# quantummind/mpi_opt

Measured on AMD Instinct MI355X. Metric: EI candidates/sec (GP/EI ask step, N=200 obs, D=10, fp64), higher is better.
Workload: dtype f64; 1 GPU; BASELINE configs[1]: GP/EI ask step, 200 observations, 10-dim, 1000000 candidates per GPU, top-5 (skopt argsort[:n_restarts]); n_obs=200, dims=10, candidates_per_gpu=1000000, parallelism=candidates sharded, 1 GPU(s), all-gather of (value,index)

## Files before the change

mpi_opt_amd/csrc/gp.hip:

```cpp

#include "mpo_internal.h"

#include <algorithm>
#include <cmath>
#include <cstdlib>
#include <string>

namespace {

typedef double f64x4 __attribute__((ext_vector_type(4)));

constexpr double kSqrt5 = 2.236067977499789696409173668731276235;
constexpr double kSqrt1_2 = 0.707106781186547524400844362104849039;
constexpr double kSqrt2Pi = 2.506628274631000502415765284811045253;
constexpr double kJitter = 1e-10;

__device__ __forceinline__ double matern52(double r, double amp) {
    const double k = r * kSqrt5;
    return amp * ((1.0 + k + k * k * (1.0 / 3.0)) * exp(-k));
}

__device__ __forceinline__ double fma_sc(double a, double b, double c) {
    double r;
    asm("v_fma_f64 %0, %1, %2, %3" : "=v"(r) : "v"(a), "v"(b), "s"(c));
// ... 146 lines not shown
        double xx = 0.0;
        for (int c = 0; c < d; ++c) xx = fma(xs[(size_t)i * dp + c], xs[(size_t)i * dp + c], xx);
        for (int c = 0; c < dp; ++c)
            xb[(size_t)i * dp + c] = c < d ? -2.0 * xs[(size_t)i * dp + c] : c == d ? 1.0 : c == d + 1 ? xx : 0.0;
        if (!(xx <= kDistNorm)) atomicOr(&bad, 1);
    }
    __syncthreads();
    if (threadIdx.x == 0) xb[(size_t)rows * dp] = bad ? 0.0 : 1.0;
}

__global__ __launch_bounds__(256) void xb_check_kernel(const double* __restrict__ mqd, const double* __restrict__ mqm,
                                                       const double* __restrict__ alpha, int n, double amp,
                                                       double* __restrict__ flag) {
    __shared__ int bad;
    __shared__ double red[4];
    if (threadIdx.x == 0) bad = 0;
    double sa = 0.0;
    for (int i = threadIdx.x; i < n; i += 256) sa += fabs(alpha[i]);
    for (int o = 32; o > 0; o >>= 1) sa += __shfl_down(sa, o, 64);
    if ((threadIdx.x & 63) == 0) red[threadIdx.x >> 6] = sa;
    __syncthreads();
    const double mu_scale = amp * (red[0] + red[1] + red[2] + red[3]);
    for (int i = threadIdx.x; i < n; i += 256) {
        const double mud = mqd[2 * i], qd = mqd[2 * i + 1], mum = mqm[2 * i], qm = mqm[2 * i + 1];
        const bool ok = fabs(qm - qd) <= 1e-10 * fmax(amp - qd, 1e-300) && fabs(mum - mud) <= 1e-10 * mu_scale;
        if (!ok) atomicOr(&bad, 1);
    }
    __syncthreads();
    if (threadIdx.x == 0 && bad) flag[0] = 0.0;
}

__global__ void kernel_matrix_unscaled_kernel(const double* __restrict__ X, int n, int d,
                                              const double* __restrict__ ls, double amp,
                                              double diag_add, double* __restrict__ K, int ldk) {
    const int j = blockIdx.x * blockDim.x + threadIdx.x;
    const int i = blockIdx.y;
    if (j >= n) return;
    double r2 = 0.0;
    for (int c = 0; c < d; ++c) {
        const double t = X[(size_t)i * d + c] / ls[c] - X[(size_t)j * d + c] / ls[c];
        r2 += t * t;
    }
    double v = matern52(sqrt(r2), amp);
    if (i == j) v += diag_add;
    K[(size_t)i * ldk + j] = v;
}

__global__ __launch_bounds__(1024) void chol_kernel(double* __restrict__ A, int n, int lda,
                                                    int32_t* __restrict__ info) {
    __shared__ int fail;
    const int tid = threadIdx.x, nt = blockDim.x;
    const int lane = tid & 63, wave = tid >> 6, nwave = nt >> 6;
    if (tid == 0) fail = 0;
    __syncthreads();
    for (int j = 0; j < n; ++j) {
        if (tid == 0) {
            const double djj = A[(size_t)j * lda + j];
            if (!(djj > 0.0) || !isfinite(djj)) fail = j + 1;
            else A[(size_t)j * lda + j] = sqrt(djj);
        }
        __syncthreads();
        if (fail) break;
        const double ljj = A[(size_t)j * lda + j];
        for (int i = j + 1 + tid; i < n; i += nt) A[(size_t)i * lda + j] /= ljj;
        __syncthreads();
        for (int i = j + 1 + wave; i < n; i += nwave) {
            const double lij = A[(size_t)i * lda + j];
            for (int k = j + 1 + lane; k <= i; k += 64)
                A[(size_t)i * lda + k] -= lij * A[(size_t)k * lda + j];
        }
        __syncthreads();
    }
    if (tid == 0) *info = fail;
}

__global__ __launch_bounds__(64) void trsm_kernel(const double* __restrict__ L, int n, int lda,
                                                  double* __restrict__ B, int nrhs, int ldb,
                                                  int trans, int cb) {
    extern __shared__ __attribute__((aligned(16))) double xsol[];
    const int lc = threadIdx.x;
    const int col = blockIdx.x * cb + lc;
    const bool active = lc < cb && col < nrhs;
    if (!active) return;
    if (!trans) {
        for (int i = 0; i < n; ++i) {
            double s = B[(size_t)i * ldb + col];
            const double* Li = L + (size_t)i * lda;
            for (int k = 0; k < i; ++k) s -= Li[k] * xsol[k * cb + lc];
            const double x = s / Li[i];
            xsol[i * cb + lc] = x;
            B[(size_t)i * ldb + col] = x;
        }
    } else {
        for (int i = n - 1; i >= 0; --i) {
            double s = B[(size_t)i * ldb + col];
            for (int k = i + 1; k < n; ++k) s -= L[(size_t)k * lda + i] * xsol[k * cb + lc];
            const double x = s / L[(size_t)i * lda + i];
            xsol[i * cb + lc] = x;
            B[(size_t)i * ldb + col] = x;
        }
    }
}

constexpr int kStreamSlack = 2;
inline size_t wfrag_elems(int np16) {
    const size_t T = np16 / 16;
    return (T * (T + 1) / 2 + 4 * kStreamSlack) * 256;
}
inline size_t wmeta_elems(int np16) {
    const int T = np16 / 16;
    return (size_t)4 * (T + 4) + T + 4;
}

__global__ void wave_plan_kernel(int T, int32_t* __restrict__ meta) {
    if (threadIdx.x != 0 || blockIdx.x != 0) return;
    int load[4] = {0, 0, 0, 0}, cnt[4] = {0, 0, 0, 0};
    for (int jt = T - 1; jt >= 0; --jt) {
        int w = 0;
        for (int v = 1; v < 4; ++v)
            if (load[v] < load[w]) w = v;
        meta[w * (T + 4) + 3 + cnt[w]++] = jt;
        load[w] += jt + 1;
    }
    int off = 0;
    for (int w = 0; w < 4; ++w) {
        int32_t* r = meta + w * (T + 4);
        r[0] = off;
        r[1] = load[w];
        r[2] = cnt[w];
        for (int t = cnt[w]; t <= T; ++t) r[3 + t] = 0;
        int g = off;
        for (int t = 0; t < cnt[w]; ++t) {
            meta[4 * (T + 4) + r[3 + t]] = g;
            g += r[3 + t] + 1;
        }
        off += load[w] + kStreamSlack;
    }
}

__global__ void pack_wfrag_kernel(const double* __restrict__ W, int n, int ldw, int T,
                                  const int32_t* __restrict__ meta, double* __restrict__ wfrag) {
    const int jt = blockIdx.y;
    if (jt >= T) return;
    const int nks = 4 * (jt + 1);
    const int e = blockIdx.x * blockDim.x + threadIdx.x;
    if (e >= nks * 64) return;
    const int ks = e >> 6, l = e & 63;
    const int i = 4 * ks + (l >> 4), j = 16 * jt + (l & 15);
    const double v = (i < n && j < n && i <= j) ? W[(size_t)j * ldw + i] : 0.0;
    wfrag[(size_t)meta[4 * (T + 4) + jt] * 256 + e] = v;
}

constexpr int kBM = 16;

struct ScoreArgs {
    int n, np16, T, d;
    double amp, y_mean, y_std;
    const double* xs;
    const double* xb;
    const double* xb_ok;
    const double* ls;
    const double* alpha;
    const double* wfrag;
    const int32_t* wmeta;
    const double* cand;
    long long m;
    double y_opt, xi, kappa;
    unsigned flags;
    int ei_positive;
    int dbg;
    double* mu;
    double* sd;
    double* vals;
    int k;
    long long* part_idx;
    double* part_val;
    double* mq;
    int panel;
    double* part;
};

__device__ __attribute__((noinline)) void score_finish_group(const ScoreArgs& a, bool valid, long long gm, double mu_n,
                                                   double q, int lane, double* tk_val, long long* tk_idx) {
    double mu = 0.0, sd = 0.0, vei = 0.0, vpi = 0.0, vlcb = 0.0;
    if (valid && (a.dbg & 8)) {
        mu = mu_n;
        sd = q;
    } else if (valid) {
        double var = a.amp - q;
        if (var < 0.0) var = 0.0;
        sd = sqrt(var) * a.y_std;
        mu = a.y_std * mu_n + a.y_mean;
        if (sd > 0.0) {
            const double improve = a.y_opt - a.xi - mu;
            const double scaled = improve / sd;
            const double cdf = ndtr(scaled);
            vei = -(improve * cdf + sd * norm_pdf(scaled));
            vpi = -cdf;
        } else {
            vei = -0.0;
            vpi = -0.0;
        }
        vlcb = mu - a.kappa * sd;
        if (a.mu) a.mu[gm] = mu;
        if (a.sd) a.sd[gm] = sd;
        if (a.vals) {
            if (a.flags & MPO_ACQ_EI) a.vals[gm] = a.ei_positive ? -vei : vei;
            if (a.flags & MPO_ACQ_PI) a.vals[a.m + gm] = vpi;
            if (a.flags & MPO_ACQ_LCB) a.vals[2 * a.m + gm] = vlcb;
        }
    }
    if (a.k <= 0 || (a.dbg & 4)) return;
    const double inf = __builtin_huge_val();
    const long long big = 0x7fffffffffffffffLL;
    const int k = a.k;
#pragma unroll
    for (int acq = 0; acq < 3; ++acq) {
        if (!(a.flags & (1u << acq))) continue;
        const double v = valid ? (acq == 0 ? vei : (acq == 1 ? vpi : vlcb)) : inf;
        const long long idx = valid ? gm : big;
        double* lv = tk_val + acq * MPO_TOPK_MAX;
        long long* li = tk_idx + acq * MPO_TOPK_MAX;
        bool cand = valid && lex_less(v, idx, lv[k - 1], li[k - 1]);
        while (__any(cand)) {
            double bv = cand ? v : inf;
            long long bi = cand ? idx : big;
            wave_lex_min(bv, bi);
            if (lane == 0) {
                int pos = k - 1;
                while (pos > 0 && lex_less(bv, bi, lv[pos - 1], li[pos - 1])) {
                    lv[pos] = lv[pos - 1];
                    li[pos] = li[pos - 1];
                    --pos;
                }
                lv[pos] = bv;
                li[pos] = bi;
            }
            asm volatile("s_waitcnt lgkmcnt(0)" ::: "memory");
            cand = cand && idx != bi && lex_less(v, idx, lv[k - 1], li[k - 1]);
        }
    }
}

__device__ __forceinline__ void score_finish_own_rows(double* kc, int wave, int lane) {
    constexpr int BM = kBM;
    __syncthreads();
    const ScoreArgs* ap = (const ScoreArgs*)__builtin_amdgcn_kernarg_segment_ptr();
    asm volatile("" : "+s"(ap));
    const ScoreArgs& f = *ap;
    double* tk_val = kc + wave * 3 * MPO_TOPK_MAX;
    long long* tk_idx = reinterpret_cast<long long*>(kc + 4 * 3 * MPO_TOPK_MAX) + wave * 3 * MPO_TOPK_MAX;
    if (lane < 3 * MPO_TOPK_MAX) {
        tk_val[lane] = __builtin_huge_val();
        tk_idx[lane] = 0x7fffffffffffffffLL;
    }
    asm volatile("s_waitcnt lgkmcnt(0)" ::: "memory");
    const long long ntl = ((f.m + BM - 1) / BM - blockIdx.x + gridDim.x - 1) / gridDim.x;
    for (long long c0 = (long long)wave * 64; c0 < ntl * BM; c0 += 256) {
        const long long cl = c0 + lane;
        const long long gm = (blockIdx.x + (cl >> 4) * (long long)gridDim.x) * BM + (cl & 15);
        const bool valid = cl < ntl * BM && gm < f.m;
        double2 v = {0.0, 0.0};
        if (valid) v = *reinterpret_cast<const double2*>(f.mq + 2 * gm);
        score_finish_group(f, valid, gm, v.x, v.y, lane, tk_val, tk_idx);
    }
    if (f.k > 0 && lane < 3 * f.k) {
        const int acq = lane / f.k, r = lane - acq * f.k;
        const size_t part = (size_t)blockIdx.x * 4 + wave;
        f.part_val[(part * 3 + acq) * f.k + r] = tk_val[acq * MPO_TOPK_MAX + r];
        f.part_idx[(part * 3 + acq) * f.k + r] = tk_idx[acq * MPO_TOPK_MAX + r];
    }
}

#define MPO_LD(D, P, OFF) asm volatile("global_load_dwordx2 %0, %1, off offset:" #OFF : "=v"(D) : "v"(P) : "memory")
#define MPO_LD4(B, P) { MPO_LD(B[0], P, 0); MPO_LD(B[1], P, 512); MPO_LD(B[2], P, 1024); MPO_LD(B[3], P, 1536); }
#define MPO_MFMA4(AP, B0, B1, B2, B3)                                                              \
    acc0 = __builtin_amdgcn_mfma_f64_16x16x4f64((AP)[0], B0, acc0, 0, 0, 0);                       \
    acc1 = __builtin_amdgcn_mfma_f64_16x16x4f64((AP)[64], B1, acc1, 0, 0, 0);                      \
    acc0 = __builtin_amdgcn_mfma_f64_16x16x4f64((AP)[128], B2, acc0, 0, 0, 0);                     \
    acc1 = __builtin_amdgcn_mfma_f64_16x16x4f64((AP)[192], B3, acc1, 0, 0, 0);
#define MPO_EI_PAIR(XC, AC, LI)                                                                    \
    {                                                                                              \
        double r2 = kR2Floor;                                                                      \
        _Pragma("unroll") for (int q = 0; q < D; ++q) {                                            \
            const double t = c[q] - XC[q];                                                         \
            r2 = fma(t, t, r2);                                                                    \
        }                                                                                          \
        const double kv = matern52_unit(r2);                         \
        mu_acc = fma(kv, AC, mu_acc);                                                              \
        kc[(size_t)((LI) >> 2) * 64 + row + ((LI) & 3) * 16] = kv;                                 \
    }

template <int DP, int D, int OCC, int MD, int FIN>
__global__ __launch_bounds__(256, OCC) void gp_score_kernel(ScoreArgs a) {
    static_assert(!MD || D + 2 <= DP, "the MFMA distance needs two spare columns");
    constexpr int BM = kBM;
    constexpr int S = 16;
    constexpr int EPT = (BM * DP + 255) / 256;
    extern __shared__ __attribute__((aligned(16))) double smem[];
    const int np16 = a.np16;
    double* kc = smem;
    double* cs = kc + (size_t)np16 * BM;
    double* red = cs + BM * DP;
    int32_t* mls = reinterpret_cast<int32_t*>(red + S * BM);

    const int tid = threadIdx.x, lane = tid & 63;
    const int wave = __builtin_amdgcn_readfirstlane(tid >> 6);
    const long long ntiles = (a.m + BM - 1) / BM;

    for (int e = tid; e < 4 * (a.T + 4); e += 256) mls[e] = a.wmeta[e];

    const bool xb_ok = MD && *a.xb_ok != 0.0;
    double raw[EPT], ls_e[EPT];
#pragma unroll
    for (int u = 0; u < EPT; ++u) {
        const int c = (tid + 256 * u) % DP;
        ls_e[u] = c < a.d ? a.ls[c] : 1.0;
    }
#define MPO_LOAD_TILE(TILE)                                                                    \
    _Pragma("unroll") for (int u = 0; u < EPT; ++u) {                                          \
        const int e = tid + 256 * u, r = e / DP, c = e % DP;                                   \
        const long long gm = (TILE) * BM + r;                                                  \
        raw[u] = (e < BM * DP && gm < a.m && c < a.d) ? __builtin_nontemporal_load(a.cand + gm * a.d + c) : 0.0; \
    }
    MPO_LOAD_TILE((long long)blockIdx.x)
    __syncthreads();
    int fw = 0;
    {
        int lw = 0;
        for (int q = 1; q < 4; ++q)
            if (mls[q * (a.T + 4) + 1] < mls[lw * (a.T + 4) + 1]) lw = q;
        fw = __builtin_amdgcn_readfirstlane((lw - (int)blockIdx.x) & 3);
    }

    const int sw = (wave + (int)blockIdx.x) & 3;
    const int32_t* mw = mls + sw * (a.T + 4);
    const int G = (a.dbg & 1) ? 0 : __builtin_amdgcn_readfirstlane(mw[1]);
    const double* bs = a.wfrag + (size_t)__builtin_amdgcn_readfirstlane(mw[0]) * 256 + lane;

    for (long long tile = blockIdx.x; tile < ntiles; tile += gridDim.x) {
    const long long m0 = tile * BM;

#pragma unroll
    for (int u = 0; u < EPT; ++u)
        if (tid + 256 * u < BM * DP) cs[tid + 256 * u] = raw[u] / ls_e[u];
    MPO_LOAD_TILE(tile + gridDim.x)
    __syncthreads();

    {
        const int row = lane & 15;
        const int slot = wave * 4 + (lane >> 4);
        double c[D];
#pragma unroll
        for (int q = 0; q < D; ++q) c[q] = cs[row * DP + q];
        double mu_acc = 0.0;
        bool md = false;
        if constexpr (MD) {
            double cc = 0.0;
#pragma unroll
            for (int q = 0; q < D; ++q) cc = fma(c[q], c[q], cc);
            md = xb_ok && __all(cc <= kDistNorm);
            if (md && !(a.dbg & 2)) {
                const int kr = lane >> 4;
                double af[DP / 4];
#pragma unroll
                for (int s = 0; s < DP / 4; ++s) {
                    const int kk = 4 * s + kr;
                    const double v = cs[row * DP + kk];
                    af[s] = kk == D ? cc : kk == D + 1 ? 1.0 : v;
                }
                const int T16 = np16 >> 4;
                const double* xbl = a.xb + (size_t)(lane & 15) * DP + kr;
                double bq[DP / 4];
                double mu4[4] = {0.0, 0.0, 0.0, 0.0};
                for (int t = wave; t < T16; t += 4) {
#pragma unroll
                    for (int s = 0; s < DP / 4; ++s) bq[s] = xbl[(size_t)t * 16 * DP + 4 * s];
                    f64x4 acc = {0.0, 0.0, 0.0, 0.0};
#pragma unroll
                    for (int s = 0; s < DP / 4; ++s) acc = __builtin_amdgcn_mfma_f64_16x16x4f64(af[s], bq[s], acc, 0, 0, 0);
                    const int i = t * 16 + (lane & 15);
                    const double al = a.alpha[i];
#pragma unroll
                    for (int r = 0; r < 4; ++r) {
                        const double kv = matern52_unit(fmax(acc[r], kR2Floor));
                        kc[(size_t)(i >> 2) * 64 + kr + 4 * r + (i & 3) * 16] = kv;
                        mu4[r] = fma(kv, al, mu4[r]);
                    }
                }
#pragma unroll
                for (int r = 0; r < 4; ++r) mu4[r] = colsum16(mu4[r]);
                if ((lane & 15) == 0) {
#pragma unroll
                    for (int r = 0; r < 4; ++r)
#pragma unroll
                        for (int q = 0; q < 4; ++q) red[(wave * 4 + q) * BM + kr + 4 * r] = q == 0 ? mu4[r] : 0.0;
                }
            }
        }
        if (md && !(a.dbg & 2)) {
        } else if (a.dbg & 2) {
            for (int i = slot; i < np16; i += S) kc[(size_t)(i >> 2) * 64 + row + (i & 3) * 16] = c[0];
        } else {
            for (int i = slot; i < np16; i += S) {
                const double* xr = a.xs + (size_t)i * DP;
                MPO_EI_PAIR(xr, a.alpha[i], i)
            }
        }
        if (!md || (a.dbg & 2)) red[slot * BM + row] = mu_acc;
    }
    __syncthreads();
    double mu_n = 0.0;
    if (wave == fw && lane < BM) {
#pragma unroll
        for (int s = 0; s < S; ++s) mu_n += red[s * BM + lane];
        mu_n *= a.amp;
    }
    __syncthreads();

    {
        double b0[4], b1[4];
        MPO_LD4(b0, bs);
        MPO_LD4(b1, bs + 256);
        const double* bp = bs + 512;
        const double* kl = kc + lane;
        double sq[4] = {0.0, 0.0, 0.0, 0.0};
        f64x4 acc0 = {0.0, 0.0, 0.0, 0.0}, acc1 = {0.0, 0.0, 0.0, 0.0};
        int t = 0, kg = 0, tlen = __builtin_amdgcn_readfirstlane(mw[3] + 1);
#define MPO_EI_GROUP(B)                                                                            \
        {                                                                                          \
            asm volatile("s_waitcnt vmcnt(4)" : "+v"(B[0]), "+v"(B[1]), "+v"(B[2]), "+v"(B[3])); \
            const double* ap = kl + kg * 256;                                                      \
            MPO_MFMA4(ap, B[0], B[1], B[2], B[3])                                                  \
            MPO_LD4(B, bp);                                                                        \
            bp += 256;                                                                             \
            if (++kg == tlen) {                                                                    \
                _Pragma("unroll") for (int r = 0; r < 4; ++r) {                                    \
                    const double v = acc0[r] + acc1[r];                                            \
                    sq[r] = fma(v, v, sq[r]);                                                      \
                }                                                                                  \
                acc0 = f64x4{0.0, 0.0, 0.0, 0.0};                                                  \
                acc1 = f64x4{0.0, 0.0, 0.0, 0.0};                                                  \
                kg = 0;                                                                            \
                tlen = __builtin_amdgcn_readfirstlane(mw[3 + (++t)] + 1);                          \
            }                                                                                      \
        }
        for (int g = 0; g < G; g += 2) {
            MPO_EI_GROUP(b0)
            if (g + 1 >= G) break;
            MPO_EI_GROUP(b1)
        }
        asm volatile("s_waitcnt vmcnt(0)" : "+v"(b0[0]), "+v"(b0[1]), "+v"(b0[2]), "+v"(b0[3]), "+v"(b1[0]),
                     "+v"(b1[1]), "+v"(b1[2]), "+v"(b1[3]));
#undef MPO_EI_GROUP
#pragma unroll
        for (int r = 0; r < 4; ++r) {
            const double v = colsum16(sq[r]);
            if ((lane & 15) == 0) red[wave * BM + (lane >> 4) + 4 * r] = v;
        }
    }
    __syncthreads();

    if (wave == fw && lane < BM && m0 + lane < a.m) {
        const double q = (red[0 * BM + lane] + red[1 * BM + lane] + red[2 * BM + lane] + red[3 * BM + lane]) *
                         (a.amp * a.amp);
        *reinterpret_cast<double2*>(a.mq + 2 * (m0 + lane)) = double2{mu_n, q};
    }
    }
    if constexpr (FIN) score_finish_own_rows(kc, wave, lane);
#undef MPO_LOAD_TILE
}

template <int DP, int D>
__global__ __launch_bounds__(256) void gp_score_streamed_kernel(ScoreArgs a) {
    constexpr int BM = kBM;
    constexpr int S = 16;
    static_assert(4 * 3 * MPO_TOPK_MAX * 16 <= 16 * kBM * 8, "the finish's top-k lists live in the smallest panel");
    extern __shared__ __attribute__((aligned(16))) double smem[];
    const int T = a.T, PT = a.panel >> 4;
    double* kc = smem;
    double* cs = kc + (size_t)a.panel * BM;
    double* red = cs + BM * DP;
    int32_t* toff = reinterpret_cast<int32_t*>(red + (S + 4) * BM);

    const int tid = threadIdx.x, lane = tid & 63;
    const int wave = __builtin_amdgcn_readfirstlane(tid >> 6);
    const long long ntiles = (a.m + BM - 1) / BM;
    const int row = lane & 15;
    const int slot = wave * 4 + (lane >> 4);
    double* part = a.part + (size_t)blockIdx.x * (size_t)(T > PT ? T - PT : 0) * 256 + lane;

    for (int e = tid; e < T; e += 256) toff[e] = a.wmeta[4 * (T + 4) + e];

    for (long long tile = blockIdx.x; tile < ntiles; tile += gridDim.x) {
        const long long m0 = tile * BM;
        for (int e = tid; e < BM * DP; e += 256) {
            const int r = e / DP, c = e % DP;
            const long long gm = m0 + r;
            cs[e] = (gm < a.m && c < a.d) ? __builtin_nontemporal_load(a.cand + gm * a.d + c) / a.ls[c] : 0.0;
        }
        __syncthreads();
        double c[D];
#pragma unroll
        for (int q = 0; q < D; ++q) c[q] = cs[row * DP + q];
        double mu_acc = 0.0;
        double sq[4] = {0.0, 0.0, 0.0, 0.0};

        for (int t0 = 0; t0 < T; t0 += PT) {
            const int t1 = min(T, t0 + PT);
            for (int i = t0 * 16 + slot; i < t1 * 16; i += S) {
                const double* xr = a.xs + (size_t)i * DP;
                const int li = i - t0 * 16;
                MPO_EI_PAIR(xr, a.alpha[i], li)
            }
            __syncthreads();
            for (int jt = t0 + ((wave - t0 - (int)blockIdx.x) & 3); jt < T; jt += 4) {
                const int ng = min(jt, t1 - 1) - t0 + 1;
                f64x4 acc0 = {0.0, 0.0, 0.0, 0.0}, acc1 = {0.0, 0.0, 0.0, 0.0};
                double* pr = part + (size_t)(jt - PT) * 256;
                if (t0 > 0) {
#pragma unroll
                    for (int r = 0; r < 4; ++r) acc0[r] = pr[r * 64];
                }
                const double* bp = a.wfrag + ((size_t)__builtin_amdgcn_readfirstlane(toff[jt]) + t0) * 256 + lane;
                const double* ap = kc + lane;
#define MPO_ST_LD(B, G)                                                                        \
                {                                                                              \
                    const double* p = bp + (size_t)min((G), ng - 1) * 256;                     \
                    MPO_LD4(B, p)                                                              \
                }
#define MPO_ST_GROUP(B, G)                                                                     \
                {                                                                              \
                    asm volatile("s_waitcnt vmcnt(8)" : "+v"(B[0]), "+v"(B[1]), "+v"(B[2]), "+v"(B[3]));  \
                    const double* q = ap + (size_t)(G) * 256;                                  \
                    MPO_MFMA4(q, B[0], B[1], B[2], B[3])                                       \
                    MPO_ST_LD(B, (G) + 3)                                                      \
                }
                const int rem = ng % 3;
                double b0[4], b1[4], b2[4];
                MPO_ST_LD(b0, rem)
                MPO_ST_LD(b1, rem + 1)
                MPO_ST_LD(b2, rem + 2)
                for (int g = 0; g < rem; ++g) {
                    const double* p = bp + (size_t)g * 256;
                    const double* q = ap + (size_t)g * 256;
                    MPO_MFMA4(q, p[0], p[64], p[128], p[192])
                }
                for (int g = rem; g < ng; g += 3) {
                    MPO_ST_GROUP(b0, g)
                    MPO_ST_GROUP(b1, g + 1)
                    MPO_ST_GROUP(b2, g + 2)
                }
                asm volatile("s_waitcnt vmcnt(0)" : "+v"(b0[0]), "+v"(b0[1]), "+v"(b0[2]), "+v"(b0[3]), "+v"(b1[0]),
                             "+v"(b1[1]), "+v"(b1[2]), "+v"(b1[3]), "+v"(b2[0]), "+v"(b2[1]), "+v"(b2[2]), "+v"(b2[3]));
#undef MPO_ST_GROUP
#undef MPO_ST_LD
                if (jt < t1) {
#pragma unroll
                    for (int r = 0; r < 4; ++r) {
                        const double v = acc0[r] + acc1[r];
                        sq[r] = fma(v, v, sq[r]);
                    }
                } else {
#pragma unroll
                    for (int r = 0; r < 4; ++r) pr[r * 64] = acc0[r] + acc1[r];
                }
            }
            __syncthreads();
        }

        red[slot * BM + row] = mu_acc;
#pragma unroll
        for (int r = 0; r < 4; ++r) {
            const double v = colsum16(sq[r]);
            if ((lane & 15) == 0) red[(S + wave) * BM + (lane >> 4) + 4 * r] = v;
        }
        __syncthreads();
        if (wave == 0 && lane < BM && m0 + lane < a.m) {
            double mu_n = 0.0;
#pragma unroll
            for (int s = 0; s < S; ++s) mu_n += red[s * BM + lane];
            mu_n *= a.amp;
            const double q = (red[(S + 0) * BM + lane] + red[(S + 1) * BM + lane] + red[(S + 2) * BM + lane] +
                              red[(S + 3) * BM + lane]) * (a.amp * a.amp);
            *reinterpret_cast<double2*>(a.mq + 2 * (m0 + lane)) = double2{mu_n, q};
        }
    }

    score_finish_own_rows(kc, wave, lane);
}
#undef MPO_EI_PAIR
#undef MPO_MFMA4
#undef MPO_LD4
#undef MPO_LD

__global__ __launch_bounds__(256) void topk_merge_kernel(const long long* __restrict__ part_idx,
                                                         const double* __restrict__ part_val,
                                                         int nparts, int chunk, int k, unsigned flags,
                                                         long long* __restrict__ out_idx,
                                                         double* __restrict__ out_val,
                                                         int out_stride, int final_stage) {
    __shared__ double lv[256 * MPO_TOPK_MAX];
    __shared__ long long li[256 * MPO_TOPK_MAX];
    const int acq = blockIdx.y;
    if (!(flags & (1u << acq))) return;
    const int tid = threadIdx.x;
    const double inf = __builtin_huge_val();
    const long long big = 0x7fffffffffffffffLL;
    const int p0 = blockIdx.x * chunk;
    const int p1 = min(nparts, p0 + chunk);
    double bv[MPO_TOPK_MAX];
    long long bi[MPO_TOPK_MAX];
#pragma unroll
    for (int r = 0; r < MPO_TOPK_MAX; ++r) { bv[r] = inf; bi[r] = big; }
    const long long total = (long long)(p1 - p0) * k;
    for (long long e = tid; e < total; e += 256) {
        const long long blk = p0 + e / k, r = e % k;
        const size_t off = ((size_t)blk * 3 + acq) * k + r;
        double v = part_val[off];
        long long i = part_idx[off];
#pragma unroll
        for (int s = 0; s < MPO_TOPK_MAX; ++s) {
            if (s < k && lex_less(v, i, bv[s], bi[s])) {
                const double tv = bv[s];
                const long long ti = bi[s];
                bv[s] = v; bi[s] = i; v = tv; i = ti;
            }
        }
    }
#pragma unroll
    for (int r = 0; r < MPO_TOPK_MAX; ++r) { lv[tid * MPO_TOPK_MAX + r] = bv[r]; li[tid * MPO_TOPK_MAX + r] = bi[r]; }
    __syncthreads();
    if (tid >= 64) return;
    int ptr[4] = {0, 0, 0, 0};
    for (int r = 0; r < k; ++r) {
        double v = inf;
        long long i = big;
        int src = -1;
#pragma unroll
        for (int q = 0; q < 4; ++q) {
            const int lst = tid + 64 * q;
            if (ptr[q] < k) {
                const double w = lv[lst * MPO_TOPK_MAX + ptr[q]];
                const long long j = li[lst * MPO_TOPK_MAX + ptr[q]];
                if (lex_less(w, j, v, i)) { v = w; i = j; src = q; }
            }
        }
        double gv = v;
        long long gi = i;
        wave_lex_min(gv, gi);
        if (src >= 0 && gi == i && gv == v) {
#pragma unroll
            for (int q = 0; q < 4; ++q) if (q == src) ptr[q]++;
        }
        if (tid == 0) {
            if (final_stage) {
                out_val[acq * out_stride + r] = gv;
                out_idx[acq * out_stride + r] = gi == big ? -1 : gi;
            } else {
                out_val[((size_t)blockIdx.x * 3 + acq) * k + r] = gv;
                out_idx[((size_t)blockIdx.x * 3 + acq) * k + r] = gi;
            }
        }
    }
}

__global__ void argmax_from_topk_kernel(const long long* __restrict__ topk_idx, long long* __restrict__ argmax) {
    *argmax = topk_idx[0];
}

#define MPO_SCORE_DIMS(X) X(4, 4) X(8, 5) X(8, 8) X(12, 10) X(12, 12) X(16, 16) X(32, 32)

inline int pad_dims(int d) {
#define MPO_X(DP, D) if (d <= DP) return DP;
    MPO_SCORE_DIMS(MPO_X)
#undef MPO_X
    return -1;
}

constexpr size_t kMaxLds = 160 * 1024;
constexpr int kMergeGroups = 256;
constexpr int kScoreGridCap = 8 * 256;

size_t score_lds_bytes(int dp, int np16) {
    const int T = np16 / 16;
    return ((size_t)np16 * kBM + (size_t)kBM * dp + 16 * kBM) * sizeof(double) + (size_t)4 * (T + 4) * sizeof(int32_t);
}

bool score_fits(int dp, int np16) { return score_lds_bytes(dp, np16) <= kMaxLds; }

constexpr size_t kStreamPartCap = (size_t)48 << 20;

size_t streamed_lds_bytes(int dp, int np16, int panel) {
    return ((size_t)panel * kBM + (size_t)kBM * dp + 20 * kBM) * sizeof(double) + (size_t)(np16 / 16) * sizeof(int32_t);
}

int streamed_grid_cap(int dp, int np16, int panel) {
    const int per_cu = (int)std::min<size_t>(8, kMaxLds / streamed_lds_bytes(dp, np16, panel));
    int cap = std::min(kScoreGridCap, std::max(1, per_cu) * 256);
    const size_t slice = (size_t)(np16 - panel) * kBM * sizeof(double);
    if (slice) cap = (int)std::min<size_t>(cap, std::max<size_t>(1, kStreamPartCap / slice));
    return cap;
}

struct ScorePlan {
    int path;
    int panel;
    size_t lds;
    int grid_cap;
    size_t part_elems;
};

int score_plan(const char* who, const MpoGpModel* model, int64_t m, ScorePlan* plan) {
    const int n = model->n, dp = model->dp, np16 = model->np16;
    auto refuse = [&](int rc) {
        if (who)
            mpo::set_error(rc == MPO_ENOTSUP
                               ? "%s: n=%d exceeds the supported maximum of %d observations"
                               : "%s: malformed model (n=%d) or MPO_GP_PANEL (a multiple of 16, >= 16; max n %d)",
                           who, n, mpo::kMaxObs);
        return rc;
    };
    if (n <= 0 || np16 < n || np16 - n >= 16 || (np16 & 15) || dp <= 0 || pad_dims(dp) != dp)
        return refuse(MPO_EINVAL);
    if (n > mpo::kMaxObs) return refuse(MPO_ENOTSUP);
    const char* e = getenv("MPO_GP_SCORE");
    const bool forced = e && std::string(e) == "streamed";
    if (!forced && score_fits(dp, np16)) {
        *plan = ScorePlan{0, 0, score_lds_bytes(dp, np16), kScoreGridCap, 0};
        return MPO_OK;
    }
    int p = np16;
    while (p > 16 && streamed_lds_bytes(dp, np16, p) > kMaxLds) p -= 16;
    if (const char* pe = getenv("MPO_GP_PANEL"); pe && *pe) {
        char* end = nullptr;
        const long v = strtol(pe, &end, 10);
        if (*end || v < 16 || v % 16) return refuse(MPO_EINVAL);
        p = (int)std::min<long>(p, v);
    }
    const int cap = streamed_grid_cap(dp, np16, p);
    const int64_t grid = std::min<int64_t>((m + kBM - 1) / kBM, cap);
    *plan = ScorePlan{1, p, streamed_lds_bytes(dp, np16, p), cap, (size_t)grid * (size_t)(np16 - p) * kBM};
    return MPO_OK;
}

using ScoreKernel = void (*)(ScoreArgs);

hipError_t launch_looped(ScoreKernel kern, const ScoreArgs& a, int ntiles, size_t lds, int cap, hipStream_t s,
                         int* grid_out) {
    const void* fn = reinterpret_cast<const void*>(kern);
    hipFuncAttributes fa;
    if (hipFuncGetAttributes(&fa, fn) != hipSuccess || fa.localSizeBytes != 0) return hipErrorInvalidDeviceFunction;
    (void)hipFuncSetAttribute(fn, hipFuncAttributeMaxDynamicSharedMemorySize, (int)lds);
    int dev = 0, cus = 0, per_cu = 0;
    (void)hipGetDevice(&dev);
    (void)hipDeviceGetAttribute(&cus, hipDeviceAttributeMultiprocessorCount, dev);
    (void)hipOccupancyMaxActiveBlocksPerMultiprocessor(&per_cu, fn, 256, lds);
    const int grid = std::max(1, std::min(std::min(ntiles, cap), std::max(1, per_cu) * std::max(1, cus)));
    if (grid_out) *grid_out = grid;
    hipLaunchKernelGGL(kern, dim3(grid), dim3(256), lds, s, a);
    return hipGetLastError();
}

template <int DP, int D, int OCC, int MD, int FIN>
bool spill_free() {
    static int ok = -1;
    if (ok < 0) {
        hipFuncAttributes fa;
        ok = hipFuncGetAttributes(&fa, reinterpret_cast<const void*>(gp_score_kernel<DP, D, OCC, MD, FIN>)) ==
                 hipSuccess &&
             fa.localSizeBytes == 0;
    }
// ... 782 lines not shown
```

Before: 759.4 million candidates/s.

## Cut per-tile barriers by double-buffering mu reduction and staging next tile early

Restructures the persistent score kernel loop so the next candidate tile is staged into shared memory right after the kernel-row phase, and the loads run two tiles ahead. The mean partial sums are reduced within a wave using shuffles and written into alternating double-buffered slots, with the q sums moved to a separate area. This removes two of the four __syncthreads per tile, and the wave-to-slot mapping now rotates across tiles. In exchange it uses more registers and adds some risk from the buffer aliasing in the reshuffled shared-memory layout.

```diff
diff --git a/mpi_opt_amd/csrc/gp.hip b/mpi_opt_amd/csrc/gp.hip
--- a/mpi_opt_amd/csrc/gp.hip
+++ b/mpi_opt_amd/csrc/gp.hip
@@ -472,6 +472,7 @@
     double* kc = smem;
     double* cs = kc + (size_t)np16 * BM;
     double* red = cs + BM * DP;
+    double* redq = red + 2 * 4 * BM;
     int32_t* mls = reinterpret_cast<int32_t*>(red + S * BM);
 
     const int tid = threadIdx.x, lane = tid & 63;
@@ -493,7 +494,12 @@
         const long long gm = (TILE) * BM + r;                                                  \
         raw[u] = (e < BM * DP && gm < a.m && c < a.d) ? __builtin_nontemporal_load(a.cand + gm * a.d + c) : 0.0; \
     }
+#define MPO_STAGE_TILE                                                                         \
+    _Pragma("unroll") for (int u = 0; u < EPT; ++u)                                            \
+        if (tid + 256 * u < BM * DP) cs[tid + 256 * u] = raw[u] / ls_e[u];
     MPO_LOAD_TILE((long long)blockIdx.x)
+    MPO_STAGE_TILE
+    MPO_LOAD_TILE((long long)blockIdx.x + gridDim.x)
     __syncthreads();
     int fw = 0;
     {
@@ -508,18 +514,15 @@
     const int G = (a.dbg & 1) ? 0 : __builtin_amdgcn_readfirstlane(mw[1]);
     const double* bs = a.wfrag + (size_t)__builtin_amdgcn_readfirstlane(mw[0]) * 256 + lane;
 
+    int vs = (wave + (int)blockIdx.x) & 3;
+    double* redm = red;
+
     for (long long tile = blockIdx.x; tile < ntiles; tile += gridDim.x) {
     const long long m0 = tile * BM;
 
-#pragma unroll
-    for (int u = 0; u < EPT; ++u)
-        if (tid + 256 * u < BM * DP) cs[tid + 256 * u] = raw[u] / ls_e[u];
-    MPO_LOAD_TILE(tile + gridDim.x)
-    __syncthreads();
-
     {
         const int row = lane & 15;
-        const int slot = wave * 4 + (lane >> 4);
+        const int slot = vs * 4 + (lane >> 4);
         double c[D];
 #pragma unroll
         for (int q = 0; q < D; ++q) c[q] = cs[row * DP + q];
@@ -543,7 +546,7 @@
                 const double* xbl = a.xb + (size_t)(lane & 15) * DP + kr;
                 double bq[DP / 4];
                 double mu4[4] = {0.0, 0.0, 0.0, 0.0};
-                for (int t = wave; t < T16; t += 4) {
+                for (int t = vs; t < T16; t += 4) {
 #pragma unroll
                     for (int s = 0; s < DP / 4; ++s) bq[s] = xbl[(size_t)t * 16 * DP + 4 * s];
                     f64x4 acc = {0.0, 0.0, 0.0, 0.0};
@@ -562,9 +565,7 @@
                 for (int r = 0; r < 4; ++r) mu4[r] = colsum16(mu4[r]);
                 if ((lane & 15) == 0) {
 #pragma unroll
-                    for (int r = 0; r < 4; ++r)
-#pragma unroll
-                        for (int q = 0; q < 4; ++q) red[(wave * 4 + q) * BM + kr + 4 * r] = q == 0 ? mu4[r] : 0.0;
+                    for (int r = 0; r < 4; ++r) redm[vs * BM + kr + 4 * r] = mu4[r];
                 }
             }
         }
@@ -577,16 +578,16 @@
                 MPO_EI_PAIR(xr, a.alpha[i], i)
             }
         }
-        if (!md || (a.dbg & 2)) red[slot * BM + row] = mu_acc;
-    }
-    __syncthreads();
-    double mu_n = 0.0;
-    if (wave == fw && lane < BM) {
-#pragma unroll
-        for (int s = 0; s < S; ++s) mu_n += red[s * BM + lane];
-        mu_n *= a.amp;
-    }
-    __syncthreads();
+        if (!md || (a.dbg & 2)) {
+            mu_acc += __shfl_xor(mu_acc, 16);
+            mu_acc += __shfl_xor(mu_acc, 32);
+            if (lane < BM) redm[vs * BM + row] = mu_acc;
+        }
+    }
+    __syncthreads();
+
+    MPO_STAGE_TILE
+    MPO_LOAD_TILE(tile + 2 * (long long)gridDim.x)
 
     {
         double b0[4], b1[4];
@@ -626,18 +627,25 @@
 #pragma unroll
         for (int r = 0; r < 4; ++r) {
             const double v = colsum16(sq[r]);
-            if ((lane & 15) == 0) red[wave * BM + (lane >> 4) + 4 * r] = v;
+            if ((lane & 15) == 0) redq[wave * BM + (lane >> 4) + 4 * r] = v;
         }
     }
     __syncthreads();
 
     if (wave == fw && lane < BM && m0 + lane < a.m) {
-        const double q = (red[0 * BM + lane] + red[1 * BM + lane] + red[2 * BM + lane] + red[3 * BM + lane]) *
+        double mu_n = 0.0;
+#pragma unroll
+        for (int s = 0; s < 4; ++s) mu_n += redm[s * BM + lane];
+        mu_n *= a.amp;
+        const double q = (redq[0 * BM + lane] + redq[1 * BM + lane] + redq[2 * BM + lane] + redq[3 * BM + lane]) *
                          (a.amp * a.amp);
         *reinterpret_cast<double2*>(a.mq + 2 * (m0 + lane)) = double2{mu_n, q};
     }
+    vs = (vs + 1) & 3;
+    redm = redm == red ? red + 4 * BM : red;
     }
     if constexpr (FIN) score_finish_own_rows(kc, wave, lane);
+#undef MPO_STAGE_TILE
 #undef MPO_LOAD_TILE
 }
 
```

New measurement: 779.6 million candidates/s, median of 6. 2.7% higher.
